# petabi/petal-neighbors

Hardware: NVIDIA B200
Metric: knn_queries_per_sec_k10 (higher is better)
Workload: dtype f32

## Files before the change

### petal-neighbors_b200/csrc/tc_filter.cuh

```cuda
#pragma once
#include <cuda.h>
#include <cuda_fp16.h>
#include <cuda_runtime.h>
#include <stdint.h>

#include "kernels.cuh"
#include "tc_prune.cuh"

namespace petal {
namespace tc {

#ifdef PN_TC_PROFILE
#define PROF_DECL unsigned pt_ = (unsigned)clock(), pc_[6] = {0, 0, 0, 0, 0, 0}
#define PROF_ADD(i) do { unsigned n_ = (unsigned)clock(); pc_[i] += n_ - pt_; pt_ = n_; } while (0)
#define PROF_FLUSH(base) do { for (int i_ = 0; i_ < 6; ++i_) atomicAdd(&a.counters[8 + (base) + i_], (unsigned long long)pc_[i_]); } while (0)
#else
#define PROF_DECL
#define PROF_ADD(i)
#define PROF_FLUSH(base)
#endif
#if defined(PN_TC_PROFILE) && defined(PN_TC_TRACE)
#define TRACE(role, tile, ev) do { if (a.trace && blockIdx.x == 0 && (tile) >= a.trace_t0 && (tile) < a.trace_t0 + 64u) a.trace[(((role) * 64) + ((tile) - a.trace_t0)) * 4 + (ev)] = clock64(); } while (0)
#else
#define TRACE(role, tile, ev)
#endif

constexpr int BM = 128;
constexpr int BN = 128;
constexpr int KC = 32;
constexpr int CHUNK_BYTES = BN * KC * 2;
constexpr int A_CHUNK_BYTES = BM * KC * 2;
constexpr int NSLOT = 6;

__device__ __forceinline__ uint32_t smem_u32(const void* p) { return (uint32_t)__cvta_generic_to_shared(p); }

__device__ __forceinline__ void mbar_init(uint64_t* bar, uint32_t count) {
    asm volatile("mbarrier.init.shared::cta.b64 [%0], %1;" ::"r"(smem_u32(bar)), "r"(count));
}
__device__ __forceinline__ void mbar_expect_tx(uint64_t* bar, uint32_t bytes) {
    asm volatile("mbarrier.arrive.expect_tx.shared::cta.b64 _, [%0], %1;" ::"r"(smem_u32(bar)), "r"(bytes) : "memory");
}
__device__ __forceinline__ void mbar_arrive(uint64_t* bar) {
    asm volatile("mbarrier.arrive.shared::cta.b64 _, [%0];" ::"r"(smem_u32(bar)) : "memory");
}
__device__ __forceinline__ void mbar_wait(uint64_t* bar, uint32_t parity) {
    asm volatile(
        "{\n\t"
        ".reg .pred P1;\n\t"
        "WAIT_LOOP:\n\t"
        "mbarrier.try_wait.parity.shared::cta.b64 P1, [%0], %1, %2;\n\t"
        "@P1 bra DONE;\n\t"
        "bra WAIT_LOOP;\n\t"
        "DONE:\n\t"
        "}" ::"r"(smem_u32(bar)), "r"(parity), "r"(1000000u) : "memory");
}
__device__ __forceinline__ void tma_load_2d(const CUtensorMap* map, uint64_t* bar, void* dst, int c0, int c1) {
    asm volatile(
        "cp.async.bulk.tensor.2d.shared::cluster.global.mbarrier::complete_tx::bytes [%0], [%1, {%3, %4}], [%2];" ::"r"(
            smem_u32(dst)),
        "l"(map), "r"(smem_u32(bar)), "r"(c0), "r"(c1)
        : "memory");
}
__device__ __forceinline__ void bulk_copy(void* dst, const void* src, uint32_t bytes, uint64_t* bar) {
    asm volatile("cp.async.bulk.shared::cluster.global.mbarrier::complete_tx::bytes [%0], [%1], %2, [%3];" ::"r"(smem_u32(dst)),
                 "l"(src), "r"(bytes), "r"(smem_u32(bar))
                 : "memory");
}
__device__ __forceinline__ bool elect_one() {
    uint32_t pred = 0;
    asm volatile("{\n\t.reg .pred px;\n\telect.sync _|px, 0xffffffff;\n\tselp.u32 %0, 1, 0, px;\n\t}" : "=r"(pred));
    return pred != 0;
}
__device__ __forceinline__ void tc_fence_before() { asm volatile("tcgen05.fence::before_thread_sync;" ::: "memory"); }
__device__ __forceinline__ void tc_fence_after() { asm volatile("tcgen05.fence::after_thread_sync;" ::: "memory"); }
__device__ __forceinline__ void tc_commit(uint64_t* bar) {
    asm volatile("tcgen05.commit.cta_group::1.mbarrier::arrive::one.shared::cluster.b64 [%0];" ::"r"(smem_u32(bar)) : "memory");
}
__device__ __forceinline__ void tc_mma_f16(uint32_t d_tmem, uint64_t adesc, uint64_t bdesc, uint32_t idesc, uint32_t accumulate) {
    asm volatile(
        "{\n\t"
        ".reg .pred p;\n\t"
        "setp.ne.b32 p, %4, 0;\n\t"
        "tcgen05.mma.cta_group::1.kind::f16 [%0], %1, %2, %3, p;\n\t"
        "}" ::"r"(d_tmem),
        "l"(adesc), "l"(bdesc), "r"(idesc), "r"(accumulate)
        : "memory");
}
__device__ __forceinline__ void tc_mma_f16_ts(uint32_t d_tmem, uint32_t a_tmem, uint64_t bdesc, uint32_t idesc, uint32_t accumulate) {
    asm volatile(
        "{\n\t"
        ".reg .pred p;\n\t"
        "setp.ne.b32 p, %4, 0;\n\t"
        "tcgen05.mma.cta_group::1.kind::f16 [%0], [%1], %2, %3, p;\n\t"
        "}" ::"r"(d_tmem),
        "r"(a_tmem), "l"(bdesc), "r"(idesc), "r"(accumulate)
        : "memory");
}
__device__ __forceinline__ void tc_cp_128x256b(uint32_t taddr, uint64_t sdesc) {
    asm volatile("tcgen05.cp.cta_group::1.128x256b [%0], %1;" ::"r"(taddr), "l"(sdesc) : "memory");
}
__device__ __forceinline__ uint64_t make_desc_sw64(uint32_t saddr) {
    return (uint64_t)((saddr >> 4) & 0x3FFF) | (1ull << 16) | (32ull << 32) | (1ull << 46) | (4ull << 61);
}
__host__ __device__ constexpr uint32_t make_idesc_f16(int M, int N) {
    return (1u << 4) | ((uint32_t)(N >> 3) << 17) | ((uint32_t)(M >> 4) << 24);
}

__device__ __forceinline__ void tmem_ld32_issue(uint32_t taddr, uint32_t (&r)[32]) {
    asm volatile(
        "tcgen05.ld.sync.aligned.32x32b.x32.b32 "
        "{%0, %1, %2, %3, %4, %5, %6, %7, %8, %9, %10, %11, %12, %13, %14, %15, "
        "%16, %17, %18, %19, %20, %21, %22, %23, %24, %25, %26, %27, %28, %29, %30, %31}, [%32];"
        : "=r"(r[0]), "=r"(r[1]), "=r"(r[2]), "=r"(r[3]), "=r"(r[4]), "=r"(r[5]), "=r"(r[6]), "=r"(r[7]), "=r"(r[8]),
          "=r"(r[9]), "=r"(r[10]), "=r"(r[11]), "=r"(r[12]), "=r"(r[13]), "=r"(r[14]), "=r"(r[15]), "=r"(r[16]),
          "=r"(r[17]), "=r"(r[18]), "=r"(r[19]), "=r"(r[20]), "=r"(r[21]), "=r"(r[22]), "=r"(r[23]), "=r"(r[24]),
          "=r"(r[25]), "=r"(r[26]), "=r"(r[27]), "=r"(r[28]), "=r"(r[29]), "=r"(r[30]), "=r"(r[31])
        : "r"(taddr)
        : "memory");
}
__device__ __forceinline__ void tmem_ld_wait(uint32_t (&r)[32]) {
    asm volatile("tcgen05.wait::ld.sync.aligned;"
                 : "+r"(r[0]), "+r"(r[1]), "+r"(r[2]), "+r"(r[3]), "+r"(r[4]), "+r"(r[5]), "+r"(r[6]), "+r"(r[7]), "+r"(r[8]),
                   "+r"(r[9]), "+r"(r[10]), "+r"(r[11]), "+r"(r[12]), "+r"(r[13]), "+r"(r[14]), "+r"(r[15]), "+r"(r[16]),
                   "+r"(r[17]), "+r"(r[18]), "+r"(r[19]), "+r"(r[20]), "+r"(r[21]), "+r"(r[22]), "+r"(r[23]), "+r"(r[24]),
                   "+r"(r[25]), "+r"(r[26]), "+r"(r[27]), "+r"(r[28]), "+r"(r[29]), "+r"(r[30]), "+r"(r[31])
                 :
                 : "memory");
}

struct SmemTopK {
    unsigned long long* sk;
    unsigned long long kth_key, floor_key;
    float t2;
    uint32_t k;
    static __device__ __forceinline__ unsigned long long make_key(float d, uint32_t i) {
        return ((unsigned long long)__float_as_uint(d) << 32) | i;
    }
    __device__ __forceinline__ void init(unsigned long long* base, int lane, uint32_t k_, bool active) {
        sk = base + lane; k = k_;
        kth_key = make_key(pos_inf<float>(), NO_ID);
        for (uint32_t s = 0; s < k; ++s) sk[s * 32] = kth_key;
        t2 = active ? pos_inf<float>() : -1.f;
        floor_key = 0ull;
    }
    __device__ __forceinline__ void set_floor(float d, uint32_t i) { floor_key = make_key(d, i) + 1ull; }
    __device__ __forceinline__ bool offer_key(unsigned long long key) {
        if (key < floor_key || key >= kth_key) return false;
        uint32_t p = k - 1;
        while (p > 0) {
            const unsigned long long pk = sk[(p - 1) * 32];
            if (key >= pk) break;
            sk[p * 32] = pk;
            --p;
        }
        sk[p * 32] = key;
        kth_key = sk[(k - 1) * 32];
        t2 = thresh2(__uint_as_float((uint32_t)(kth_key >> 32)));
        return true;
    }
    __device__ __forceinline__ void store(float* out_d, uint32_t* out_i) const {
        for (uint32_t s = 0; s < k; ++s) {
            const unsigned long long e = sk[s * 32];
            out_d[s] = __uint_as_float((uint32_t)(e >> 32)); out_i[s] = (uint32_t)e;
        }
    }
};

struct FilterArgs {
    DevTree<float> t;
    const float4* q;
    const float* q_margin;
    uint32_t nq, k;
    uint32_t row0;
    uint32_t n_tiles;
    uint32_t tiles_per_split;
    uint32_t nkc;
    uint32_t last_steps;
    uint32_t stages;
    uint32_t gs;
    float t2_scale;
    float* g_bound;
    float* part_d;
    uint32_t* part_i;
    const float* floor_d;
    const uint32_t* floor_i;
    unsigned long long* counters;
    const uint32_t* tile_bits;
    const uint32_t* tile_cnt;
    const float* seed_t2;
    uint32_t tile_words;
#ifdef PN_TC_PROFILE
    uint32_t dbg;
    long long* trace;
    uint32_t trace_t0;
#endif
};

__device__ __forceinline__ void split3_f16(float x, __half& h1, __half& h2, __half& h3) {
    h1 = __float2half_rn(x);
    const float r1 = x - __half2float(h1);
    h2 = __float2half_rn(r1);
    h3 = __float2half_rn(r1 - __half2float(h2));
}

__device__ __forceinline__ size_t baug_offset(uint32_t row, uint32_t j, uint32_t nkc) {
    const uint32_t tile = row / BN, r = row % BN, c = j / KC, e = j % KC;
    return ((size_t)(tile * nkc + c) * BN + r) * KC + (((e >> 3) ^ ((r >> 1) & 3u)) << 3) + (e & 7u);
}
__global__ void build_baug_kernel(const float* __restrict__ pts, const float* __restrict__ center, float scale, uint32_t n,
                                  uint32_t d, uint32_t dpad, uint32_t kp, __half* __restrict__ baug, unsigned int* pmax_bits) {
    const uint32_t i = blockIdx.x * blockDim.x + threadIdx.x;
    if (i >= n) return;
    const float* p = pts + (size_t)i * dpad;
    const uint32_t nkc = kp / KC;
    float nrm = 0.f;
    for (uint32_t j = 0; j < d; ++j) {
        const float v = (p[j] - center[j]) * scale;
        nrm = nrm + v * v;
        baug[baug_offset(i, j, nkc)] = __float2half_rn(-2.0f * v);
    }
    for (uint32_t j = d + NSLOT; j < kp; ++j) baug[baug_offset(i, j, nkc)] = __float2half_rn(0.f);
    __half h1, h2, h3;
    split3_f16(nrm, h1, h2, h3);
    const __half one = __float2half_rn(1.f);
    baug[baug_offset(i, d, nkc)] = one;     baug[baug_offset(i, d + 1, nkc)] = one; baug[baug_offset(i, d + 2, nkc)] = one;
    baug[baug_offset(i, d + 3, nkc)] = h1;  baug[baug_offset(i, d + 4, nkc)] = h2;  baug[baug_offset(i, d + 5, nkc)] = h3;
    atomicMax(pmax_bits, __float_as_uint(sqrtf(nrm) * 1.000001f));
}

__global__ void build_aaug_kernel(const float* __restrict__ q, const float* __restrict__ center, float scale, uint32_t nq,
                                  uint32_t d, uint32_t dpad, uint32_t kp, float pmax, __half* __restrict__ aaug,
                                  float* __restrict__ q_margin) {
    const uint32_t i = blockIdx.x * blockDim.x + threadIdx.x;
    if (i >= nq) return;
    const float* p = q + (size_t)i * dpad;
    __half* o = aaug + (size_t)i * kp;
    float nrm = 0.f;
    for (uint32_t j = 0; j < d; ++j) {
        const float v = (p[j] - center[j]) * scale;
        nrm = nrm + v * v;
    }
    const float qn = sqrtf(nrm) * 1.000001f;
    const bool in_range = qn <= 200.f;
    for (uint32_t j = 0; j < d; ++j) o[j] = __float2half_rn(in_range ? (p[j] - center[j]) * scale : 0.f);
    for (uint32_t j = d + NSLOT; j < kp; ++j) o[j] = __float2half_rn(0.f);
    __half h1, h2, h3;
    split3_f16(in_range ? nrm : 0.f, h1, h2, h3);
    const __half one = __float2half_rn(1.f);
    o[d] = h1; o[d + 1] = h2; o[d + 2] = h3; o[d + 3] = one; o[d + 4] = one; o[d + 5] = one;
    const float sn = qn + pmax;
    const float e = 1.01f * 0.001953125f * qn * pmax + 6.2e-05f * sqrtf((float)d) * (qn + 2.f * pmax) +
                    (float)(kp + 8) * 4.76837158203125e-07f * sn * sn;
    q_margin[i] = in_range ? e : pos_inf<float>();
}

template <int DVR, int K, int MT, int NUM_ACC, bool SHARED, int SW = BN, bool PRUNE = false>
__global__ void __launch_bounds__((5 * MT + 2) * 32, 1)
knn_filter_kernel(const __grid_constant__ CUtensorMap map_a, const unsigned char* __restrict__ baug, const FilterArgs a) {
    extern __shared__ __align__(1024) unsigned char smem_raw[];
    unsigned char* smem = (unsigned char*)(((uintptr_t)smem_raw + 1023) & ~(uintptr_t)1023);
    unsigned char* smem_a = smem;
    unsigned char* smem_b = smem + (size_t)MT * a.nkc * A_CHUNK_BYTES;
    uint64_t* bars = reinterpret_cast<uint64_t*>(smem_b + (size_t)a.stages * a.gs * CHUNK_BYTES);
    uint64_t* full_bar = bars;
    uint64_t* empty_bar = bars + a.stages;
    uint64_t* tfull_bar = bars + 2 * a.stages;
    uint64_t* tempty_bar = tfull_bar + NUM_ACC * MT;
    uint64_t* a_bar = tempty_bar + NUM_ACC * MT;
    uint32_t* tmem_slot = reinterpret_cast<uint32_t*>(a_bar + 1);
    uint32_t* qbuf = tmem_slot + 4;
    constexpr int QWORDS = 192;
    unsigned long long* tk = reinterpret_cast<unsigned long long*>(qbuf + 4 * MT * QWORDS);

    const int warp = __shfl_sync(0xffffffffu, threadIdx.x >> 5, 0), lane = threadIdx.x & 31;
    constexpr int EPI_WARPS = 4 * MT;
    constexpr bool TS = (MT == 2 && (NUM_ACC == 1 || SW == 64)) || MT == 3;
    constexpr int TMEM_COLS = TS ? 512 : NUM_ACC * MT * SW;
    constexpr int U = BN / SW;
    static_assert(SW == BN || SW == 64, "stage width is a whole tile or half a tile");

    if (warp == EPI_WARPS && lane == 0) {
        for (uint32_t s = 0; s < a.stages; ++s) { mbar_init(&full_bar[s], 1); mbar_init(&empty_bar[s], MT); }
        for (int s = 0; s < NUM_ACC * MT; ++s) { mbar_init(&tfull_bar[s], 1); mbar_init(&tempty_bar[s], 4); }
        mbar_init(a_bar, 1);
        asm volatile("fence.mbarrier_init.release.cluster;" ::: "memory");
        asm volatile("prefetch.tensormap [%0];" ::"l"(&map_a) : "memory");
    }
    if (warp == EPI_WARPS + 1) {
        asm volatile("tcgen05.alloc.cta_group::1.sync.aligned.shared::cta.b32 [%0], %1;" ::"r"(smem_u32(tmem_slot)), "r"(TMEM_COLS) : "memory");
        asm volatile("tcgen05.relinquish_alloc_permit.cta_group::1.sync.aligned;" ::: "memory");
    }
    tc_fence_before();
    __syncthreads();
    tc_fence_after();
    const uint32_t tmem_base = __shfl_sync(0xffffffffu, *tmem_slot, 0);

    const uint32_t row_base = a.row0 + blockIdx.x * (MT * BM);
    static_assert(!(PRUNE && SHARED), "the pruned scan does not split the point stream");
    const uint32_t j_begin = PRUNE ? 0u : blockIdx.y * a.tiles_per_split;
    const uint32_t n_my = PRUNE ? a.tile_cnt[blockIdx.x] : min(a.n_tiles - j_begin, a.tiles_per_split);
    const uint32_t* my_bits = PRUNE ? a.tile_bits + (size_t)blockIdx.x * a.tile_words : nullptr;

    if (warp == EPI_WARPS || warp == EPI_WARPS + MT + 1) {
        const uint32_t pid = warp == EPI_WARPS ? 0u : 1u;
        if (lane == 0) {
            if (pid == 0) {
                mbar_expect_tx(a_bar, (uint32_t)(MT * a.nkc * A_CHUNK_BYTES));
                for (int mt = 0; mt < MT; ++mt)
                    for (uint32_t c = 0; c < a.nkc; ++c)
                        tma_load_2d(&map_a, a_bar, smem_a + (size_t)(mt * a.nkc + c) * A_CHUNK_BYTES, (int)(c * KC), (int)(row_base + mt * BM));
            }
            const uint32_t total = n_my * a.nkc;
            const uint32_t n_groups = (total + a.gs - 1) / a.gs;
            const unsigned char* bsrc = baug + (size_t)j_begin * a.nkc * CHUNK_BYTES;
            PROF_DECL;
            if (PRUNE) {
                TileIter it;
                if (n_my) it.init(my_bits);
                for (uint32_t i = 0, ch = 0; i < n_my; ++i) {
                    const uint32_t tile = it.next();
                    for (uint32_t c = 0; c < a.nkc; ++c, ++ch) {
                        const uint32_t g = ch / a.gs, gi = ch % a.gs;
                        if ((g & 1u) != pid) continue;
                        const uint32_t s = g % a.stages, ph = (g / a.stages) & 1u;
                        if (gi == 0) {
                            mbar_wait(&empty_bar[s], ph ^ 1u);
                            mbar_expect_tx(&full_bar[s], min(a.gs, total - ch) * CHUNK_BYTES);
                        }
                        bulk_copy(smem_b + (size_t)(s * a.gs + gi) * CHUNK_BYTES, baug + ((size_t)tile * a.nkc + c) * CHUNK_BYTES, CHUNK_BYTES, &full_bar[s]);
                    }
                }
            } else
            for (uint32_t g = pid; g < n_groups; g += 2) {
                const uint32_t s = g % a.stages, ph = (g / a.stages) & 1u;
                const uint32_t first = g * a.gs, cnt = min(a.gs, total - first);
                PROF_ADD(1);
                mbar_wait(&empty_bar[s], ph ^ 1u);
                PROF_ADD(0);
#ifdef PN_TC_PROFILE
                if (a.dbg & 2u) { mbar_arrive(&full_bar[s]); continue; }
#endif
                mbar_expect_tx(&full_bar[s], cnt * CHUNK_BYTES);
                bulk_copy(smem_b + (size_t)s * a.gs * CHUNK_BYTES, bsrc + (size_t)first * CHUNK_BYTES, cnt * CHUNK_BYTES, &full_bar[s]);
            }
            if (pid == 0) PROF_FLUSH(12);
        }
    } else if (warp > EPI_WARPS && warp <= EPI_WARPS + MT) {
        {
            const int mt = warp - (EPI_WARPS + 1);
            const uint64_t a_desc0 = make_desc_sw64(smem_u32(smem_a)) + (uint64_t)(mt * a.nkc * (A_CHUNK_BYTES >> 4));
            const uint64_t b_desc0 = make_desc_sw64(smem_u32(smem_b));
            const uint32_t total = n_my * a.nkc;
            mbar_wait(a_bar, 0);
            const uint32_t a_ksteps = 2 * a.nkc - (a.last_steps > 1 ? 0u : 1u);
            const uint32_t a_tmem = tmem_base + NUM_ACC * MT * SW + mt * (a_ksteps * 8);
            if (TS) {
                tc_fence_after();
                if (elect_one()) {
                    for (uint32_t c = 0; c < a.nkc; ++c) {
                        const uint64_t ad = a_desc0 + (uint64_t)(c * (A_CHUNK_BYTES >> 4));
                        tc_cp_128x256b(a_tmem + c * 16, ad);
                        if (c + 1 < a.nkc || a.last_steps > 1) tc_cp_128x256b(a_tmem + c * 16 + 8, ad + 2);
                    }
                }
                __syncwarp();
            }
            uint32_t it = 0, g = 0, gi = 0, s = 0, sph = 0;
            uint32_t u = 0;
            constexpr uint32_t idesc_u = make_idesc_f16(BM, SW);
            PROF_DECL;
            for (uint32_t j = 0; j < n_my; ++j) {
                const uint32_t it0 = it, g0 = g, gi0 = gi, s0 = s, sph0 = sph;
#pragma unroll
                for (int h = 0; h < U; ++h, ++u) {
                    if (h) { it = it0; g = g0; gi = gi0; s = s0; sph = sph0; }
                    const uint32_t as = u % NUM_ACC, aph = (u / NUM_ACC) & 1u;
                    mbar_wait(&tempty_bar[as * MT + mt], aph ^ 1u);
                    tc_fence_after();
                    PROF_ADD(0);
                    if (lane == 0) TRACE(8 + mt, j, 0);
                    const uint32_t d_tmem = tmem_base + (as * MT + mt) * SW;
                    for (uint32_t c = 0; c < a.nkc; ++c, ++it) {
                        if (gi == 0 && h == 0) {
                            mbar_wait(&full_bar[s], sph);
                            tc_fence_after();
                            PROF_ADD(1);
                        }
                        if (lane == 0 && c == 0) TRACE(8 + mt, j, 1);
                        const uint64_t bd = b_desc0 + (uint64_t)((s * a.gs + gi) * (CHUNK_BYTES >> 4) + h * (SW * KC * 2 >> 4));
                        const uint64_t ad = a_desc0 + (uint64_t)(c * (A_CHUNK_BYTES >> 4));
                        const bool last = gi + 1 == a.gs || it + 1 == total;
                        if (elect_one()) {
                            const bool two = c + 1 < a.nkc || a.last_steps > 1;
                            if (TS) {
                                tc_mma_f16_ts(d_tmem, a_tmem + c * 16, bd, idesc_u, c > 0 ? 1u : 0u);
                                if (two) tc_mma_f16_ts(d_tmem, a_tmem + c * 16 + 8, bd + 2, idesc_u, 1u);
                            } else {
                                tc_mma_f16(d_tmem, ad, bd, idesc_u, c > 0 ? 1u : 0u);
                                if (two) tc_mma_f16(d_tmem, ad + 2, bd + 2, idesc_u, 1u);
                            }
                            if (last && h == U - 1) tc_commit(&empty_bar[s]);
                        }
                        __syncwarp();
                        if (last) { gi = 0; ++g; if (++s == a.stages) { s = 0; sph ^= 1u; } } else ++gi;
                    }
                    if (elect_one()) tc_commit(&tfull_bar[as * MT + mt]);
                    __syncwarp();
                    PROF_ADD(2);
                    if (lane == 0) TRACE(8 + mt, j, 2);
                }
            }
            if (mt == 0 && lane == 0) PROF_FLUSH(0);
        }
    } else {
        const int mt = warp >> 2, quad = warp & 3;
        const uint32_t wrow0 = row_base + mt * BM + quad * 32;
        const uint32_t qrow = wrow0 + lane;
        const bool active = qrow < a.nq;
        const DevTree<float>& t = a.t;
        const int DV = DVR > 0 ? DVR : (int)t.dv;
        unsigned long long* q_ent = reinterpret_cast<unsigned long long*>(qbuf + warp * QWORDS);
        unsigned long long* x_key = q_ent + 64;
        SmemTopK topk;
        topk.init(tk + warp * (a.k * 32), lane, a.k, active);
        if (a.floor_d && active) topk.set_floor(a.floor_d[qrow], a.floor_i[qrow]);
        const float margin = active ? a.q_margin[qrow] : 0.f;
        const float t2s = a.t2_scale;
        const float seed2 = a.seed_t2 && active ? a.seed_t2[qrow] : pos_inf<float>();
        TileIter titer;
        if (PRUNE && n_my) titer.init(my_bits);
        float theta = active ? xadd(xmul(seed2, t2s), margin) : -pos_inf<float>();
        float* gb = SHARED && active ? a.g_bound + (qrow - a.row0) : nullptr;
        auto refresh_theta = [&](bool publish) {
            float b = fminf(topk.t2, seed2);
            if (SHARED && gb) {
                if (publish) atomicMin(reinterpret_cast<int*>(gb), __float_as_int(b));
                b = fminf(b, __ldcg(gb));
            }
            theta = xadd(xmul(b, t2s), margin);
        };
        const unsigned full = 0xffffffffu;
        const unsigned lt_mask = (1u << lane) - 1u;
        unsigned long long hits = 0;
        int qn = 0;

        auto drain = [&](int cnt) {
            unsigned long long key = ~0ull;
            int o = 32 + lane;
            const bool valid = lane < cnt;
            if (valid) {
                const unsigned long long e = q_ent[lane];
                o = (int)(e >> 32);
                const uint32_t prow = (uint32_t)e;
                const float4* qr = a.q + (size_t)(wrow0 + o) * DV;
                const float4* pr = t.pts + (size_t)prow * DV;
                float acc = 0.f;
                if (DVR > 0) {
#pragma unroll
                    for (int jc = 0; jc < (DVR > 0 ? DVR : 1); ++jc) acc = fold(acc, __ldg(qr + jc), __ldg(pr + jc));
                } else {
                    for (int jc = 0; jc < DV; ++jc) acc = fold(acc, __ldg(qr + jc), __ldg(pr + jc));
                }
                key = SmemTopK::make_key(xsqrt(acc), __ldg(t.ids + prow));
            }
            const unsigned grp = __match_any_sync(full, o);
            const int rank = __popc(grp & lt_mask);
            const int rounds = __reduce_max_sync(full, valid ? rank + 1 : 0);
            for (int r = 0; r < rounds; ++r) {
                const bool send = valid && rank == r;
                if (send) x_key[o] = key;
                const unsigned owners = __reduce_or_sync(full, send ? (1u << o) : 0u);
                __syncwarp();
                if ((owners >> lane) & 1u) {
                    if (topk.offer_key(x_key[lane])) refresh_theta(true);
                }
                __syncwarp();
            }
        };

        auto test32 = [&](const uint32_t (&r)[32], uint32_t j, int col0, uint32_t& bits) -> bool {
            float mb[4];
#pragma unroll
            for (int b = 0; b < 4; ++b) {
                const float x0 = fminf(__uint_as_float(r[8 * b]), fminf(__uint_as_float(r[8 * b + 1]), __uint_as_float(r[8 * b + 2])));
                const float x1 = fminf(__uint_as_float(r[8 * b + 3]), fminf(__uint_as_float(r[8 * b + 4]), __uint_as_float(r[8 * b + 5])));
                mb[b] = fminf(fminf(x0, x1), fminf(__uint_as_float(r[8 * b + 6]), __uint_as_float(r[8 * b + 7])));
            }
            const float m = fminf(fminf(mb[0], mb[1]), fminf(mb[2], mb[3]));
            bits = 0;
            if (!__any_sync(full, m <= theta)) return false;
            if (m <= theta) {
#pragma unroll
                for (int b = 0; b < 4; ++b) {
                    if (mb[b] <= theta) {
#pragma unroll
                        for (int i = 0; i < 8; ++i) bits |= (__uint_as_float(r[8 * b + i]) <= theta ? 1u : 0u) << (8 * b + i);
                    }
                }
                const int valid = (int)t.n - (int)(j * BN + col0);
                if (valid < 32) bits &= valid > 0 ? ((1u << valid) - 1u) : 0u;
            }
            return true;
        };
        auto push32 = [&](uint32_t bits, uint32_t j, int col0) {
            for (;;) {
                const bool has = bits != 0;
                const unsigned mask = __ballot_sync(full, has);
                if (!mask) break;
                if (has) {
                    const int i = __ffs(bits) - 1;
                    bits &= bits - 1;
                    const int slot = qn + __popc(mask & lt_mask);
                    const uint32_t prow = j * BN + col0 + i;
                    q_ent[slot] = (unsigned long long)prow | ((unsigned long long)lane << 32);
                    asm volatile("prefetch.global.L2 [%0];" ::"l"(t.pts + (size_t)prow * DV));
                }
                qn += __popc(mask);
                hits += __popc(mask);
                __syncwarp();
                if (qn >= 32) {
                    drain(32);
                    const int rest = qn - 32;
                    unsigned long long te = 0;
                    if (lane < rest) te = q_ent[32 + lane];
                    __syncwarp();
                    if (lane < rest) q_ent[lane] = te;
                    __syncwarp();
                    qn = rest;
                }
            }
        };

        auto scan32 = [&](const uint32_t (&r)[32], uint32_t j, int col0) {
            float mb[4];
#pragma unroll
            for (int b = 0; b < 4; ++b) {
                const float x0 = fminf(__uint_as_float(r[8 * b]), fminf(__uint_as_float(r[8 * b + 1]), __uint_as_float(r[8 * b + 2])));
                const float x1 = fminf(__uint_as_float(r[8 * b + 3]), fminf(__uint_as_float(r[8 * b + 4]), __uint_as_float(r[8 * b + 5])));
                mb[b] = fminf(fminf(x0, x1), fminf(__uint_as_float(r[8 * b + 6]), __uint_as_float(r[8 * b + 7])));
            }
            const float m = fminf(fminf(mb[0], mb[1]), fminf(mb[2], mb[3]));
            if (!__any_sync(full, m <= theta)) return;
            uint32_t bits = 0;
            if (m <= theta) {
#pragma unroll
                for (int b = 0; b < 4; ++b) {
                    if (mb[b] <= theta) {
#pragma unroll
                        for (int i = 0; i < 8; ++i) bits |= (__uint_as_float(r[8 * b + i]) <= theta ? 1u : 0u) << (8 * b + i);
                    }
                }
                const int valid = (int)t.n - (int)(j * BN + col0);
                if (valid < 32) bits &= valid > 0 ? ((1u << valid) - 1u) : 0u;
            }
            for (;;) {
                const bool has = bits != 0;
                const unsigned mask = __ballot_sync(full, has);
                if (!mask) break;
                if (has) {
                    const int i = __ffs(bits) - 1;
                    bits &= bits - 1;
                    const int slot = qn + __popc(mask & lt_mask);
                    const uint32_t prow = j * BN + col0 + i;
                    q_ent[slot] = (unsigned long long)prow | ((unsigned long long)lane << 32);
                    asm volatile("prefetch.global.L2 [%0];" ::"l"(t.pts + (size_t)prow * DV));
                }
                qn += __popc(mask);
                hits += __popc(mask);
                __syncwarp();
                if (qn >= 32) {
                    drain(32);
                    const int rest = qn - 32;
                    unsigned long long te = 0;
                    if (lane < rest) te = q_ent[32 + lane];
                    __syncwarp();
                    if (lane < rest) q_ent[lane] = te;
                    __syncwarp();
                    qn = rest;
                }
            }
        };

        if constexpr (MT <= 2 && SW == BN) {
            constexpr int G = BN / 32;
            uint32_t r[G][32];
            const uint32_t lane_off = (uint32_t)(quad * 32) << 16;
            PROF_DECL;
            for (uint32_t jr = 0; jr < n_my; ++jr) {
                const uint32_t j = PRUNE ? titer.next() : j_begin + jr;
                const uint32_t as = jr % NUM_ACC, aph = (jr / NUM_ACC) & 1u;
                PROF_ADD(3);
                mbar_wait(&tfull_bar[as * MT + mt], aph);
                tc_fence_after();
                PROF_ADD(0);
                const uint32_t taddr = tmem_base + lane_off + (as * MT + mt) * BN;
    #pragma unroll
                for (int g = 0; g < G; ++g) tmem_ld32_issue(taddr + g * 32, r[g]);
    #pragma unroll
                for (int g = 0; g < G; ++g) tmem_ld_wait(r[g]);
                tc_fence_before();
                __syncwarp();
                if (lane == 0) mbar_arrive(&tempty_bar[as * MT + mt]);
                PROF_ADD(1);
    #ifdef PN_TC_PROFILE
                if (a.dbg & 1u) continue;
    #endif
    #pragma unroll
                for (int g = 0; g < G; ++g) scan32(r[g], j, g * 32);
                PROF_ADD(2);
                if (((PRUNE ? jr : j) & 31u) == 31u) {
                    if (qn > 0) { drain(qn); qn = 0; __syncwarp(); }
                    if (SHARED && gb) refresh_theta(false);
                }
            }
            if (warp == 0 && lane == 0) PROF_FLUSH(6);
        } else if constexpr (SW < BN) {
            constexpr int G = SW / 32;
            uint32_t r[G][32];
            const uint32_t lane_off = (uint32_t)(quad * 32) << 16;
            uint32_t u = 0;
            PROF_DECL;
            for (uint32_t jr = 0; jr < n_my; ++jr) {
                const uint32_t j = PRUNE ? titer.next() : j_begin + jr;
#pragma unroll
                for (int h = 0; h < U; ++h, ++u) {
                    const uint32_t as = u % NUM_ACC, aph = (u / NUM_ACC) & 1u;
                    PROF_ADD(3);
                    mbar_wait(&tfull_bar[as * MT + mt], aph);
                    tc_fence_after();
                    PROF_ADD(0);
                    if (lane == 0 && h == 0) TRACE(warp, j, 0);
                    const uint32_t taddr = tmem_base + lane_off + (as * MT + mt) * SW;
    #pragma unroll
                    for (int g = 0; g < G; ++g) tmem_ld32_issue(taddr + g * 32, r[g]);
    #pragma unroll
                    for (int g = 0; g < G; ++g) tmem_ld_wait(r[g]);
                    tc_fence_before();
                    __syncwarp();
                    if (lane == 0) mbar_arrive(&tempty_bar[as * MT + mt]);
                    PROF_ADD(1);
                    if (lane == 0 && h == 0) TRACE(warp, j, 1);
    #ifdef PN_TC_PROFILE
                    if (a.dbg & 1u) continue;
    #endif
                    uint32_t bits[G];
                    uint32_t any = 0;
    #pragma unroll
                    for (int g = 0; g < G; ++g) any |= test32(r[g], j, (h * G + g) * 32, bits[g]) ? 1u << g : 0u;
                    if (any) {
    #pragma unroll
                        for (int g = 0; g < G; ++g)
                            if (any & (1u << g)) push32(bits[g], j, (h * G + g) * 32);
                    }
                    PROF_ADD(2);
                }
                if (lane == 0) TRACE(warp, j, 2);
                if (((PRUNE ? jr : j) & 31u) == 31u) {
                    if (qn > 0) { drain(qn); qn = 0; __syncwarp(); }
                    if (SHARED && gb) refresh_theta(false);
                }
                if (lane == 0) TRACE(warp, j, 3);
            }
            if (warp == 0 && lane == 0) PROF_FLUSH(6);
        } else {
            constexpr int H = MT > 2 ? 2 : 1;
            constexpr int G = BN / 32 / H;
            uint32_t r[G][32];
            const uint32_t lane_off = (uint32_t)(quad * 32) << 16;
            PROF_DECL;
            for (uint32_t jr = 0; jr < n_my; ++jr) {
                const uint32_t j = PRUNE ? titer.next() : j_begin + jr;
                const uint32_t as = jr % NUM_ACC, aph = (jr / NUM_ACC) & 1u;
                PROF_ADD(3);
                mbar_wait(&tfull_bar[as * MT + mt], aph);
                tc_fence_after();
                PROF_ADD(0);
                if (lane == 0) TRACE(warp, j, 0);
                const uint32_t taddr = tmem_base + lane_off + (as * MT + mt) * BN;
                uint32_t bits[H * G];
                uint32_t any = 0;
    #pragma unroll
                for (int h = 0; h < H; ++h) {
    #pragma unroll
                    for (int g = 0; g < G; ++g) tmem_ld32_issue(taddr + (h * G + g) * 32, r[g]);
    #pragma unroll
                    for (int g = 0; g < G; ++g) tmem_ld_wait(r[g]);
                    if (h == H - 1) {
                        tc_fence_before();
                        __syncwarp();
                        if (lane == 0) mbar_arrive(&tempty_bar[as * MT + mt]);
                        PROF_ADD(1);
                        if (lane == 0) TRACE(warp, j, 1);
                    }
    #ifdef PN_TC_PROFILE
                    if (a.dbg & 1u) continue;
    #endif
    #pragma unroll
                    for (int g = 0; g < G; ++g) any |= test32(r[g], j, (h * G + g) * 32, bits[h * G + g]) ? 1u << (h * G + g) : 0u;
                }
                if (any) {
    #pragma unroll
                    for (int g = 0; g < H * G; ++g)
                        if (any & (1u << g)) push32(bits[g], j, g * 32);
                }
                PROF_ADD(2);
                if (lane == 0) TRACE(warp, j, 2);
                if (((PRUNE ? jr : j) & 31u) == 31u) {
                    if (qn > 0) { drain(qn); qn = 0; __syncwarp(); }
                    if (SHARED && gb) refresh_theta(false);
                }
                if (lane == 0) TRACE(warp, j, 3);
            }
            if (warp == 0 && lane == 0) PROF_FLUSH(6);
        }
        if (qn > 0) { drain(qn); qn = 0; }
        if (active) {
            const size_t base = ((size_t)blockIdx.y * (a.nq - a.row0) + (qrow - a.row0)) * a.k;
            topk.store(a.part_d + base, a.part_i + base);
        }
        if (a.counters && lane == 0) atomicAdd(&a.counters[2], hits);
    }

    tc_fence_before();
    __syncthreads();
    if (warp == EPI_WARPS + 1) {
        tc_fence_after();
        asm volatile("tcgen05.dealloc.cta_group::1.sync.aligned.b32 %0, %1;" ::"r"(tmem_base), "r"(TMEM_COLS) : "memory");
    }
}

}
}
```

Before: 9.517 million.

## Issue all MMAs from one warp with A-collector fill/lastuse reuse for MT=4

When MT is 4, the stage width is half a tile and the TS path is off, one MMA warp issues the tcgen05 MMAs for all four M-subtiles instead of one warp per subtile. It pairs consecutive half-tile B operands so the same A descriptor is loaded into the A collector once (fill) and reused (lastuse). The half-tiles are staggered across subtiles so pairs can form. The aim is to cut shared-memory reads of A and MMA issue overhead. The cost is serialising all issue on one warp and more complex barrier accounting, with empty_bar initialised to one arrival.

```diff
diff --git a/petal-neighbors_b200/csrc/tc_filter.cuh b/petal-neighbors_b200/csrc/tc_filter.cuh
--- a/petal-neighbors_b200/csrc/tc_filter.cuh
+++ b/petal-neighbors_b200/csrc/tc_filter.cuh
@@ -82,6 +82,26 @@
         ".reg .pred p;\n\t"
         "setp.ne.b32 p, %4, 0;\n\t"
         "tcgen05.mma.cta_group::1.kind::f16 [%0], %1, %2, %3, p;\n\t"
+        "}" ::"r"(d_tmem),
+        "l"(adesc), "l"(bdesc), "r"(idesc), "r"(accumulate)
+        : "memory");
+}
+__device__ __forceinline__ void tc_mma_f16_fill(uint32_t d_tmem, uint64_t adesc, uint64_t bdesc, uint32_t idesc, uint32_t accumulate) {
+    asm volatile(
+        "{\n\t"
+        ".reg .pred p;\n\t"
+        "setp.ne.b32 p, %4, 0;\n\t"
+        "tcgen05.mma.cta_group::1.kind::f16.collector::a::fill [%0], %1, %2, %3, p;\n\t"
+        "}" ::"r"(d_tmem),
+        "l"(adesc), "l"(bdesc), "r"(idesc), "r"(accumulate)
+        : "memory");
+}
+__device__ __forceinline__ void tc_mma_f16_lastuse(uint32_t d_tmem, uint64_t adesc, uint64_t bdesc, uint32_t idesc, uint32_t accumulate) {
+    asm volatile(
+        "{\n\t"
+        ".reg .pred p;\n\t"
+        "setp.ne.b32 p, %4, 0;\n\t"
+        "tcgen05.mma.cta_group::1.kind::f16.collector::a::lastuse [%0], %1, %2, %3, p;\n\t"
         "}" ::"r"(d_tmem),
         "l"(adesc), "l"(bdesc), "r"(idesc), "r"(accumulate)
         : "memory");
@@ -278,9 +298,11 @@
     constexpr int TMEM_COLS = TS ? 512 : NUM_ACC * MT * SW;
     constexpr int U = BN / SW;
     static_assert(SW == BN || SW == 64, "stage width is a whole tile or half a tile");
+    constexpr bool REUSE = MT == 4 && SW < BN && !TS;
+    constexpr int ISSUERS = REUSE ? 1 : MT;
 
     if (warp == EPI_WARPS && lane == 0) {
-        for (uint32_t s = 0; s < a.stages; ++s) { mbar_init(&full_bar[s], 1); mbar_init(&empty_bar[s], MT); }
+        for (uint32_t s = 0; s < a.stages; ++s) { mbar_init(&full_bar[s], 1); mbar_init(&empty_bar[s], ISSUERS); }
         for (int s = 0; s < NUM_ACC * MT; ++s) { mbar_init(&tfull_bar[s], 1); mbar_init(&tempty_bar[s], 4); }
         mbar_init(a_bar, 1);
         asm volatile("fence.mbarrier_init.release.cluster;" ::: "memory");
@@ -344,6 +366,84 @@
                 bulk_copy(smem_b + (size_t)s * a.gs * CHUNK_BYTES, bsrc + (size_t)first * CHUNK_BYTES, cnt * CHUNK_BYTES, &full_bar[s]);
             }
             if (pid == 0) PROF_FLUSH(12);
+        }
+    } else if (REUSE && warp > EPI_WARPS && warp <= EPI_WARPS + MT) {
+        if (warp == EPI_WARPS + 1) {
+            const uint64_t a_desc0 = make_desc_sw64(smem_u32(smem_a));
+            const uint64_t b_desc0 = make_desc_sw64(smem_u32(smem_b));
+            const uint32_t total = n_my * a.nkc;
+            constexpr uint32_t idesc_u = make_idesc_f16(BM, SW);
+            constexpr uint32_t h1_off = SW * KC * 2 >> 4;
+            mbar_wait(a_bar, 0);
+            PROF_DECL;
+            auto slot_of = [&](uint32_t ch) { return (ch / a.gs) % a.stages * a.gs + ch % a.gs; };
+            auto issue = [&](int mt, uint32_t v0, bool pair) {
+                const uint32_t vw = pair ? v0 + 1 : v0;
+                mbar_wait(&tempty_bar[(vw & 1u) * MT + mt], ((vw >> 1) & 1u) ^ 1u);
+                tc_fence_after();
+                PROF_ADD(0);
+                const uint32_t v1 = v0 + 1;
+                const uint32_t d0 = tmem_base + ((v0 & 1u) * MT + mt) * SW, d1 = tmem_base + ((v1 & 1u) * MT + mt) * SW;
+                for (uint32_t c = 0; c < a.nkc; ++c) {
+                    const uint64_t ad = a_desc0 + (uint64_t)((mt * a.nkc + c) * (A_CHUNK_BYTES >> 4));
+                    const uint64_t b0 = b_desc0 + (uint64_t)(slot_of((v0 >> 1) * a.nkc + c) * (CHUNK_BYTES >> 4) + (v0 & 1u) * h1_off);
+                    const uint64_t b1 = b_desc0 + (uint64_t)(slot_of((v1 >> 1) * a.nkc + c) * (CHUNK_BYTES >> 4) + (v1 & 1u) * h1_off);
+                    const bool two = c + 1 < a.nkc || a.last_steps > 1;
+                    if (elect_one()) {
+                        const uint32_t acc = c > 0 ? 1u : 0u;
+                        if (pair) {
+                            tc_mma_f16_fill(d0, ad, b0, idesc_u, acc);
+                            tc_mma_f16_lastuse(d1, ad, b1, idesc_u, acc);
+                            if (two) {
+                                tc_mma_f16_fill(d0, ad + 2, b0 + 2, idesc_u, 1u);
+                                tc_mma_f16_lastuse(d1, ad + 2, b1 + 2, idesc_u, 1u);
+                            }
+                        } else {
+                            tc_mma_f16(d0, ad, b0, idesc_u, acc);
+                            if (two) tc_mma_f16(d0, ad + 2, b0 + 2, idesc_u, 1u);
+                        }
+                        if (c + 1 == a.nkc) {
+                            tc_commit(&tfull_bar[(v0 & 1u) * MT + mt]);
+                            if (pair) tc_commit(&tfull_bar[(v1 & 1u) * MT + mt]);
+                        }
+                    }
+                    __syncwarp();
+                }
+            };
+            for (uint32_t s = 0; s <= n_my; ++s) {
+                if (s < n_my) {
+                    for (uint32_t c = 0; c < a.nkc; ++c) {
+                        const uint32_t ch = s * a.nkc + c;
+                        if (ch % a.gs == 0) {
+                            const uint32_t g = ch / a.gs;
+                            mbar_wait(&full_bar[g % a.stages], (g / a.stages) & 1u);
+                            tc_fence_after();
+                        }
+                    }
+                    PROF_ADD(1);
+                }
+#pragma unroll
+                for (int mt = MT / 2; mt < MT; ++mt) {
+                    if (s > 0 && s < n_my) issue(mt, 2 * s - 1, true);
+                    else if (s > 0) issue(mt, 2 * s - 1, false);
+                    else if (s < n_my) issue(mt, 0, false);
+                }
+                if (s < n_my) {
+#pragma unroll
+                    for (int mt = 0; mt < MT / 2; ++mt) issue(mt, 2 * s, true);
+                }
+                if (s > 0) {
+                    for (uint32_t c = 0; c < a.nkc; ++c) {
+                        const uint32_t ch = (s - 1) * a.nkc + c;
+                        if (ch % a.gs == a.gs - 1 || ch + 1 == total) {
+                            if (elect_one()) tc_commit(&empty_bar[(ch / a.gs) % a.stages]);
+                            __syncwarp();
+                        }
+                    }
+                }
+                PROF_ADD(2);
+            }
+            if (lane == 0) PROF_FLUSH(0);
         }
     } else if (warp > EPI_WARPS && warp <= EPI_WARPS + MT) {
         {
```

New measurement: 4.514 million, median of 6. 52.6% lower.
